# AnastasiaBelenkii/tendermint

Hardware: AMD Instinct MI355X
Metric: ed25519 verifies/sec at 1/2/4/8 GPUs + p50 VerifyCommit latency, 150 vals (higher is better)
Workload: dtype int32

## Files before the change

__graft_entry__.py:

```python
import os
import subprocess
import sys

REPO = os.path.dirname(os.path.abspath(__file__))


def build() -> None:
    env = dict(os.environ, PYTORCH_ROCM_ARCH="gfx950")
    subprocess.run(["make", "-s", "-C", os.path.join(REPO, "tendermint_amd", "csrc")], check=True, env=env)
    subprocess.run(["bash", os.path.join(REPO, "tools", "build_checks.sh")], check=True, env=env)
    subprocess.run(["make", "-s", "-C", os.path.join(REPO, "oracle")], check=True)
    subprocess.run(["make", "-s", "-C", os.path.join(REPO, "tendermint_amd", "testing", "csrc")], check=True)
    subprocess.run(["make", "-s", "-C", os.path.join(REPO, "tests", "native")], check=True)
    subprocess.run(["make", "-s", "-C", os.path.join(REPO, "tests", "native", "secp")], check=True)
    subprocess.run(["make", "-s", "-C", os.path.join(REPO, "tests", "native", "secpcomb")], check=True)
    subprocess.run(["make", "-s", "-C", os.path.join(REPO, "tests", "native", "merkle")], check=True)
    subprocess.run(["make", "-s", "-C", os.path.join(REPO, "tests", "native", "pcache")], check=True)
    subprocess.run(["make", "-s", "-C", os.path.join(REPO, "tests", "native", "colorder")], check=True)
    subprocess.run(["make", "-s", "-C", os.path.join(REPO, "tests", "native", "split")], check=True)
    subprocess.run(["make", "-s", "-C", os.path.join(REPO, "tests", "native", "blocks")], check=True)
    subprocess.run(["make", "-s", "-C", os.path.join(REPO, "tests", "native", "voteext")], check=True)
    subprocess.run(["make", "-s", "-C", os.path.join(REPO, "tests", "native", "proofops")], check=True)
    subprocess.run(["make", "-s", "-C", os.path.join(REPO, "tests", "native", "stage")], check=True)
    subprocess.run(["make", "-s", "-C", os.path.join(REPO, "tests", "native", "results")], check=True)
    subprocess.run(["make", "-s", "-C", os.path.join(REPO, "tests", "native", "keyorder")], check=True)
    subprocess.run(["make", "-s", "-C", os.path.join(REPO, "tests", "native", "blockwire")], check=True)
    subprocess.run(["make", "-s", "-C", os.path.join(REPO, "tests", "native", "lightwire")], check=True)
    subprocess.run(["make", "-s", "-C", os.path.join(REPO, "tests", "native", "valset")], check=True)
    sys.path.insert(0, REPO)
    import tendermint_amd
    from tendermint_amd import _native
    _native.lib()


def smoke() -> None:
    sys.path.insert(0, REPO)
    sys.path.insert(0, os.path.join(REPO, "oracle"))
    import numpy as np
    import torch
    from tendermint_amd import _native
    from tendermint_amd.testing.factory import make_c2_batch
    import oracle_c

    assert torch.cuda.is_available(), "smoke() needs a GPU"
    ctx = _native.Context(1)
    b = make_c2_batch(1000, seed=7)
    ok_g, vec_g = ctx.ed25519_verify_batch(b.pk, b.sig, b.msg, b.off)
    ok_o, vec_o = oracle_c.ed25519_verify_packed(b.pk, b.sig, b.msg, b.off, threads=4)
    assert ok_g == ok_o and np.array_equal(vec_g, vec_o), "GPU validity vector differs from the oracle"
    info = _native.build_info()
    print(f"smoke ok: {int(vec_g.sum())}/{b.n} valid, bit-exact vs oracle; {info['version']} "
          f"(src digest of this tree {'matches' if info['src_match'] else 'DIFFERS: ' + info['src_digest_tree']})")


if __name__ == "__main__":
    build()
    smoke()
```

tendermint_amd/csrc/verify_kernels.hip:

```cpp
#include <hip/hip_runtime.h>
#include <cstdlib>
#include <cstring>
#include <atomic>
#include "ed25519_core.h"
#include "quad.h"
#include "sr25519_core.h"
#include "verify_kernels.h"
#include "kernel_util.h"
#include "comb.h"
#include "halfscalar.h"
#include "ktimer.h"

namespace tmv {

__global__ void __launch_bounds__(kVerifyBlock)
k_ed25519_verify(const uint8_t *__restrict__ pk, const uint8_t *__restrict__ sig,
                 const uint8_t *__restrict__ msg, const uint32_t *__restrict__ msg_off, uint32_t n,
                 const ge_precomp *__restrict__ btable, uint8_t *__restrict__ valid, int aligned) {
  const uint32_t i = blockIdx.x * blockDim.x + threadIdx.x;
  if (i >= n) return;
  uint32_t a_w[8], r_w[8], s_w[8];
  if (aligned) {
    load_words_aligned(a_w, pk + 32ull * i);
    load_words_aligned(r_w, sig + 64ull * i);
    load_words_aligned(s_w, sig + 64ull * i + 32);
  } else {
    load_words_unaligned(a_w, pk + 32ull * i);
    load_words_unaligned(r_w, sig + 64ull * i);
    load_words_unaligned(s_w, sig + 64ull * i + 32);
  }
  const uint32_t o0 = msg_off[i], o1 = msg_off[i + 1];
  const bool ok = ed25519_verify_core(a_w, r_w, s_w, msg + o0, o1 - o0, btable);
  valid[i] = ok ? 1 : 0;
}


template <bool SR>
__device__ __forceinline__ void prep_store_point(uint32_t e, bool isA, bool ok, ge_p3 &P, const Ed25519Work &w) {
  if (!ok) ge_p3_identity(P);
  w.flags[4 * e + (isA ? 0 : 1)] = ok ? 1 : 0;
  if (w.niels) {
    niels_pt np;
    fe t;
    fe_sub(t, P.Y, P.X); fe_carry(np.ypx, t);
    fe_add(t, P.Y, P.X); fe_carry(np.ymx, t);
    fe_mul(t, P.T, consts::d2()); fe_neg(np.xy2d, t);
    np.pad[0] = np.pad[1] = 0;
    niels_store(w.niels, 2ull * e + (isA ? 1 : 0), np);
  }
  fe *dst = (isA ? w.negA : w.Rc) + 4ull * e;
  if (isA || SR) {
    fe t;
    if (isA) fe_neg(t, P.X); else t = P.X;
    dst[0] = t;
    dst[1] = P.Y;
    fe_one(t); dst[2] = t;
    if (isA) fe_neg(t, P.T); else t = P.T;
    dst[3] = t;
  } else {
    ge_cached c;
    ge_p3_to_cached(c, P);
    fe t;
    fe_carry(t, c.YmX); dst[0] = t;
    fe_carry(t, c.YpX); dst[1] = t;
    dst[2] = c.T2d;
    dst[3] = c.Z;
  }
}

template <bool SR>
__device__ __forceinline__ void prep_decode_block(uint32_t bx, const uint8_t *__restrict__ pk,
                                                  const uint8_t *__restrict__ sig, const uint32_t *__restrict__ idx,
                                                  const uint32_t *count_ptr, uint32_t n, Ed25519Work w, int aligned) {
  const uint32_t m = entry_count(count_ptr, n);
  const uint32_t j = bx * blockDim.x + threadIdx.x;
  if (j >= 2 * m) return;
  const bool isA = j < m;
  const uint32_t e = isA ? j : j - m;
  const uint32_t i = idx ? idx[e] : e;
  uint32_t p_w[8];
  const uint8_t *src = isA ? pk + 32ull * i : sig + 64ull * i;
  if (aligned) load_words_aligned(p_w, src);
  else load_words_unaligned(p_w, src);
  ge_p3 P;
  bool ok;
  if (SR) ok = ristretto_decode(P, p_w);
  else ok = ge_decode_zip215(P, p_w);
  prep_store_point<SR>(e, isA, ok, P, w);
}

template <bool SR>
__device__ __forceinline__ void prep_hash_block(uint32_t bx, const uint8_t *__restrict__ pk,
                                                const uint8_t *__restrict__ sig, const uint8_t *__restrict__ msg,
                                                const uint32_t *__restrict__ msg_off, const uint32_t *__restrict__ idx,
                                                const uint32_t *count_ptr, uint32_t n, Ed25519Work w,
                                                const strobe_t *__restrict__ prefix, int aligned) {
  const uint32_t m = entry_count(count_ptr, n);
  const uint32_t e = bx * blockDim.x + threadIdx.x;
  if (e >= m) return;
  const uint32_t i = idx ? idx[e] : e;
  uint32_t a_w[8], r_w[8];
  if (aligned) {
    load_words_aligned(a_w, pk + 32ull * i);
    load_words_aligned(r_w, sig + 64ull * i);
  } else {
    load_words_unaligned(a_w, pk + 32ull * i);
    load_words_unaligned(r_w, sig + 64ull * i);
  }
  uint32_t k[8];
  const uint32_t o0 = msg_off[i], o1 = msg_off[i + 1];
  if constexpr (SR) {
    __shared__ uint64_t strobe_lanes[25][kVerifyBlock];
    sr25519_challenge_lds<kVerifyBlock>(k, *prefix, &strobe_lanes[0][threadIdx.x], a_w, r_w, msg + o0, o1 - o0);
  } else {
    uint32_t h[16];
    sha512_pq_msg(h, r_w, a_w, msg + o0, o1 - o0);
    sc_reduce512(k, h);
  }
  uint4 *kd = reinterpret_cast<uint4 *>(w.k + 8ull * e);
  kd[0] = make_uint4(k[0], k[1], k[2], k[3]);
  kd[1] = make_uint4(k[4], k[5], k[6], k[7]);
  if (w.hs) {
    uint32_t u[4], v[4];
    bool neg = false;
    const bool fast = half::reduce(u, neg, v, k);
    uint4 *hd = reinterpret_cast<uint4 *>(w.hs + 12ull * e);
    hd[0] = make_uint4(u[0], u[1], u[2], u[3]);
    hd[1] = make_uint4(v[0], v[1], v[2], v[3]);
    hd[2] = make_uint4((fast ? 1u : 0u) | (neg ? 2u : 0u), 0u, 0u, 0u);
  }
}

template <bool SR>
__global__ void __launch_bounds__(kVerifyBlock)
k_prep_fused(const uint8_t *__restrict__ pk, const uint8_t *__restrict__ sig, const uint8_t *__restrict__ msg,
             const uint32_t *__restrict__ msg_off, const uint32_t *__restrict__ idx, const uint32_t *count_ptr,
             uint32_t n, Ed25519Work w, const strobe_t *__restrict__ prefix, int aligned, uint32_t dblocks) {
  if (blockIdx.x < dblocks) prep_decode_block<SR>(blockIdx.x, pk, sig, idx, count_ptr, n, w, aligned);
  else prep_hash_block<SR>(blockIdx.x - dblocks, pk, sig, msg, msg_off, idx, count_ptr, n, w, prefix, aligned);
}

__global__ void __launch_bounds__(kVerifyBlock)
k_prep_probe(const uint8_t *__restrict__ pk, const uint8_t *__restrict__ sig, const uint8_t *__restrict__ msg,
             const uint32_t *__restrict__ msg_off, const uint32_t *__restrict__ idx, uint32_t n, Ed25519Work w,
             int aligned, uint32_t rblocks, uint32_t hblocks) {
  if (blockIdx.x < rblocks) {
    const uint32_t e = blockIdx.x * blockDim.x + threadIdx.x;
    if (e >= n) return;
    const uint32_t i = idx ? idx[e] : e;
    uint32_t r_w[8];
    if (aligned) load_words_aligned(r_w, sig + 64ull * i);
    else load_words_unaligned(r_w, sig + 64ull * i);
    ge_p3 P;
    const bool ok = ge_decode_zip215(P, r_w);
    prep_store_point<false>(e, false, ok, P, w);
    return;
  }
  if (blockIdx.x < rblocks + hblocks) {
    prep_hash_block<false>(blockIdx.x - rblocks, pk, sig, msg, msg_off, idx, nullptr, n, w, nullptr, aligned);
    return;
  }
  const uint32_t e = (blockIdx.x - rblocks - hblocks) * blockDim.x + threadIdx.x;
  const bool live = e < n;
  bool hit = false;
  if (live) {
    const uint32_t i = idx ? idx[e] : e;
    uint32_t a_w[8];
    if (aligned) load_words_aligned(a_w, pk + 32ull * i);
    else load_words_unaligned(a_w, pk + 32ull * i);
    ge_p3 P;
    hit = pc_probe(P, w.pc.table, w.pc.bucket_mask, a_w);
    if (hit) prep_store_point<false>(e, true, true, P, w);
  }
  const uint32_t lane = threadIdx.x & 63;
  const uint64_t hm = __ballot(hit), mm = __ballot(live && !hit);
  uint32_t base = 0;
  if (lane == 0) {
    if (hm) atomicAdd(&w.pc.counters[0], (unsigned long long)__popcll(hm));
    if (mm) {
      atomicAdd(&w.pc.counters[1], (unsigned long long)__popcll(mm));
      base = atomicAdd(w.miss_count, (uint32_t)__popcll(mm));
    }
  }
  if (mm) {
    base = __shfl(base, 0);
    if (live && !hit) w.miss_list[base + __popcll(mm & ((1ull << lane) - 1))] = e;
  }
}

constexpr int kMissBlock = 64;
__global__ void __launch_bounds__(kMissBlock)
k_prep_miss(const uint8_t *__restrict__ pk, const uint32_t *__restrict__ idx, uint32_t n, Ed25519Work w,
            int aligned) {
  const uint32_t cnt = min(*w.miss_count, n);
  if (blockIdx.x * kMissBlock >= cnt) return;
  const uint32_t t = blockIdx.x * kMissBlock + threadIdx.x;
  if (t >= cnt) return;
  const uint32_t e = w.miss_list[t];
  if (e >= n) return;
  const uint32_t i = idx ? idx[e] : e;
  uint32_t a_w[8];
  if (aligned) load_words_aligned(a_w, pk + 32ull * i);
  else load_words_unaligned(a_w, pk + 32ull * i);
  ge_p3 P;
  const bool ok = ge_decode_zip215(P, a_w);
  if (ok) pc_insert(w.pc.table, w.pc.bucket_mask, a_w, P.X);
  prep_store_point<false>(e, true, ok, P, w);
}

constexpr int kQuadSigs = kQuadBlock / 4;

constexpr int kDigV = 0, kDigB = 64, kDigU = 96, kDigBytes = 128;

TMV_DEV void quad_multiples(fe *tab, const fe &P) {
  const int c = threadIdx.x & 3;
  fe r, Pm, Q, Q0;
  quad::to_cached(Q0, P);
  tab[0 * 4 + c] = Q0;
  quad::dbl(r, P);
  quad::p1p1_to_p3(Pm, r);
  quad::to_cached(Q, Pm);
  tab[1 * 4 + c] = Q;
  for (int t = 2; t < 8; t++) {
    quad::add(r, Pm, Q0);
    quad::p1p1_to_p3(Pm, r);
    quad::to_cached(Q, Pm);
    tab[t * 4 + c] = Q;
  }
}

template <bool SR>
TMV_DEV void neg_r_p3(fe &P, const fe &Rc) {
  const int c = threadIdx.x & 3;
  if (SR) {
    if (c == 0 || c == 3) fe_neg(P, Rc);
    else P = Rc;
    return;
  }
  fe o, t, K;
  quad::fe_dpp<quad::qp(1, 0, 3, 2)>(o, Rc);
  if (c == 0) fe_sub(t, Rc, o);
  else if (c == 1) fe_add(t, Rc, o);
  else t = o;
  if (c == 3) {
    const uint32_t w[8] = {0x323607aau, 0xda1f0d89u, 0xbd86abd1u, 0xf4a22967u,
                           0x32463099u, 0xd4e9deebu, 0xeb2a31bcu, 0x3f6f812du};
    fe_from_words(K, w);
  } else {
    fe_zero(K);
    K.v[0] = c == 2 ? 2 : 1;
  }
  quad::qmul(P, t, K);
}

template <bool SR, bool GT>
__device__ __forceinline__ void quad_block(uint32_t blk, fe *tab_lds, int8_t (*dig)[kDigBytes],
                                           const uint8_t *__restrict__ sig, const uint32_t *__restrict__ idx,
                                           const uint32_t *count_ptr, uint32_t n, const Ed25519Work &w,
                                           const fe *__restrict__ btab_q, uint8_t *__restrict__ out, int aligned,
                                           const uint8_t *__restrict__ group_ok, uint32_t group_log2,
                                           const uint8_t *__restrict__ sub_ok,
                                           const uint32_t *__restrict__ fail_list,
                                           const uint32_t *__restrict__ fail_count,
                                           const uint32_t *__restrict__ fb_list, uint32_t nl, int half_on) {
  const uint32_t m = entry_count(count_ptr, n);
  const int c = threadIdx.x & 3;
  const int q = threadIdx.x >> 2;
  uint32_t b0 = 0, e;
  bool live;
  if (fb_list) {
    if (blk * kQuadSigs >= nl) return;
    const uint32_t t = blk * kQuadSigs + q;
    live = t < nl;
    e = fb_list[live ? t : nl - 1];
  } else {
    if (fail_list) {
      const uint32_t per_log2 = group_log2 - 4;
      if (blk >= (*fail_count << per_log2)) return;
      b0 = (fail_list[blk >> per_log2] << group_log2) + ((blk & ((1u << per_log2) - 1)) << 4);
    } else {
      b0 = blk * kQuadSigs;
    }
    if (b0 >= m) return;
    const uint32_t raw = b0 + q;
    live = raw < m;
    e = live ? raw : m - 1;
  }
  const uint32_t i = idx ? idx[e] : e;
  bool pass = false;
  if (group_ok && !fb_list) {
    pass = !fail_list && group_ok[b0 >> group_log2];
    if (!pass && sub_ok) {
      pass = true;
      for (uint32_t s = b0 >> kSubGroupLog2; s <= (b0 + kQuadSigs - 1) >> kSubGroupLog2; s++) pass = pass && sub_ok[s];
    }
  }
  if (pass) {
    if (!live || c != 0) return;
    uint32_t s_raw[8], s_w[8];
    if (aligned) load_words_aligned(s_raw, sig + 64ull * i + 32);
    else load_words_unaligned(s_raw, sig + 64ull * i + 32);
    bool s_ok;
    if (SR) {
      s_ok = sr25519_decode_s(s_w, s_raw);
    } else {
      s_ok = sc_is_canonical(s_raw);
    }
    const bool a_ok = w.flags[4 * e] != 0;
    const bool r_ok = w.flags[4 * e + 1] != 0;
    const int status = SR ? (!a_ok ? -1 : (!s_ok ? -2 : (r_ok ? 1 : 0))) : ((a_ok && r_ok && s_ok) ? 1 : 0);
    out[i] = (uint8_t)(int8_t)status;
    return;
  }

  uint32_t s_raw[8], s_w[8];
  if (aligned) load_words_aligned(s_raw, sig + 64ull * i + 32);
  else load_words_unaligned(s_raw, sig + 64ull * i + 32);
  bool s_ok;
  if (SR) {
    s_ok = sr25519_decode_s(s_w, s_raw);
  } else {
#pragma unroll
    for (int t = 0; t < 8; t++) s_w[t] = s_raw[t];
    s_ok = sc_is_canonical(s_w);
  }
  if (!s_ok) s_w[7] &= 0x0fffffffu;
  bool fast, neg_u;
  {
    uint32_t k_w[8];
    const uint4 *kp = reinterpret_cast<const uint4 *>(w.k + 8ull * e);
    const uint4 k0 = kp[0], k1 = kp[1];
    k_w[0] = k0.x; k_w[1] = k0.y; k_w[2] = k0.z; k_w[3] = k0.w;
    k_w[4] = k1.x; k_w[5] = k1.y; k_w[6] = k1.z; k_w[7] = k1.w;
    half::Scalars sc;
    if (half_on == 1 && w.hs) {
      const uint4 *hp = reinterpret_cast<const uint4 *>(w.hs + 12ull * e);
      const uint4 hu = hp[0], hv = hp[1], hf = hp[2];
      const uint32_t u4[4] = {hu.x, hu.y, hu.z, hu.w}, v4[4] = {hv.x, hv.y, hv.z, hv.w};
      half::scalars_from(sc, u4, (hf.x & 2u) != 0, v4, (hf.x & 1u) != 0, k_w, s_w);
    } else if (half_on == 1 || (half_on == 2 && e % 3 != 0)) {
      half::scalars(sc, k_w, s_w);
    } else {
#pragma unroll
      for (int t = 0; t < 8; t++) { sc.u[t] = t == 0; sc.v[t] = k_w[t]; sc.b[t] = s_w[t]; }
      sc.fast = false;
      sc.u_neg = false;
    }
    fast = sc.fast;
    neg_u = sc.u_neg;
    if (c == 0) {
      if (fast) recode16_n<32>(&dig[q][kDigV], sc.v);
      else recode16_n<64>(&dig[q][kDigV], sc.v);
    } else if (c == 1) {
      recode256_store(&dig[q][kDigB], sc.b);
    } else if (c == 2) {
      recode16_n<32>(&dig[q][kDigU], sc.u);
    }
  }
  const bool a_ok = w.flags[4 * e] != 0;
  const bool r_ok = w.flags[4 * e + 1] != 0;

  fe *tabA = GT ? w.tabA + 64ull * e : tab_lds + q * 64;
  fe *tabR = tabA + 32;
  quad_multiples(tabA, w.negA[4ull * e + c]);
  {
    fe nR;
    neg_r_p3<SR>(nR, w.Rc[4ull * e + c]);
    quad_multiples(tabR, nR);
  }
  __syncthreads();

  fe acc, r;
  quad::p3_identity(acc);
  fe idq;
  quad::cached_identity(idq);
  const int nw = fast ? 32 : 64;
  const int nw_wave = __ballot(!fast) ? 64 : 32;
  const fe *btab_hi = btab_q + 4 * kBaseQuadEntries;
  for (int wdx = nw_wave - 1; wdx >= 0; wdx--) {
    if (wdx >= nw) continue;
    const bool even = (wdx & 1) == 0;
    const int da = dig[q][kDigV + wdx];
    const int du = wdx < 32 ? dig[q][kDigU + wdx] : 0;
    const int db = even ? dig[q][kDigB + (wdx >> 1)] : 0;
    const int dh = (even && fast) ? dig[q][kDigB + 16 + (wdx >> 1)] : 0;
    const int aa = da < 0 ? -da : da, au = du < 0 ? -du : du, ab = db < 0 ? -db : db, ah = dh < 0 ? -dh : dh;
    fe aent = tabA[(aa ? aa - 1 : 0) * 4 + c];
    fe rent = tabR[(au ? au - 1 : 0) * 4 + c];
    fe bent, hent;
    if (even) {
      bent = btab_q[(ab ? ab - 1 : 0) * 4 + c];
      if (fast) hent = btab_hi[(ah ? ah - 1 : 0) * 4 + c];
    }
    if (wdx != nw - 1) {
#pragma unroll
      for (int d = 0; d < 4; d++) {
        quad::dbl(r, acc);
        quad::p1p1_to_p3(acc, r);
      }
    }
    fe_cmov(aent, idq, aa == 0);
    quad::cached_cneg(aent, da < 0);
    quad::add(r, acc, aent);
    quad::p1p1_to_p3(acc, r);
    if (wdx < 32) {
      fe_cmov(rent, idq, au == 0);
      quad::cached_cneg(rent, (du < 0) != neg_u);
      quad::add(r, acc, rent);
      quad::p1p1_to_p3(acc, r);
    }
    if (even) {
      fe_cmov(bent, idq, ab == 0);
      quad::cached_cneg(bent, (db < 0) != neg_u);
      quad::add(r, acc, bent);
      quad::p1p1_to_p3(acc, r);
      if (fast) {
        fe_cmov(hent, idq, ah == 0);
        quad::cached_cneg(hent, (dh < 0) != neg_u);
        quad::add(r, acc, hent);
        quad::p1p1_to_p3(acc, r);
      }
    }
  }
  int status;
  if (SR) {
    const bool eq = quad::is_ristretto_identity(acc);
    status = !a_ok ? -1 : (!s_ok ? -2 : (!r_ok ? 0 : (eq ? 1 : 0)));
  } else {
    const bool ok = quad::is_identity_times8(acc) && s_ok && a_ok && r_ok;
    status = ok ? 1 : 0;
  }
  if (live && c == 0) out[i] = (uint8_t)(int8_t)status;
}


template <bool SR, bool GT>
__global__ void __launch_bounds__(kQuadBlock)
k_verify_quad(const uint8_t *__restrict__ sig, const uint32_t *__restrict__ idx, const uint32_t *count_ptr,
              uint32_t n, Ed25519Work w, const fe *__restrict__ btab_q, uint8_t *__restrict__ out, int aligned,
              const uint8_t *__restrict__ group_ok, uint32_t group_log2, const uint8_t *__restrict__ sub_ok,
              const uint32_t *__restrict__ fail_list, const uint32_t *__restrict__ fail_count,
              const uint32_t *__restrict__ fb_list, const uint32_t *__restrict__ fb_count, int half_on) {
  __shared__ fe tab_lds[GT ? 4 : kQuadSigs * 16 * 4];
  __shared__ int8_t dig[kQuadSigs][kDigBytes];
  quad_block<SR, GT>(blockIdx.x, tab_lds, dig, sig, idx, count_ptr, n, w, btab_q, out, aligned, group_ok,
                     group_log2, sub_ok, fail_list, fail_count, fb_list, fb_list ? *fb_count : 0u, half_on);
}

template <bool SR>
__global__ void __launch_bounds__(kQuadBlock)
k_verify_quad_list(const uint8_t *__restrict__ sig, const uint32_t *__restrict__ idx, const uint32_t *count_ptr,
                   uint32_t n, Ed25519Work w, const fe *__restrict__ btab_q, uint8_t *__restrict__ out,
                   int aligned, const uint32_t *__restrict__ fb_list, const uint32_t *__restrict__ fb_count,
                   int half_on) {
  __shared__ fe tab_lds[4];
  __shared__ int8_t dig[kQuadSigs][kDigBytes];
  const uint32_t nl = *fb_count;
  for (uint32_t blk = blockIdx.x; blk * kQuadSigs < nl; blk += gridDim.x) {
    quad_block<SR, true>(blk, tab_lds, dig, sig, idx, count_ptr, n, w, btab_q, out, aligned, nullptr, 0u, nullptr,
                         nullptr, nullptr, fb_list, nl, half_on);
    __syncthreads();
  }
}

__global__ void __launch_bounds__(256)
k_partition(const uint8_t *__restrict__ kind, uint32_t n, uint32_t *counts, uint32_t *idx_ed,
            uint32_t *idx_sr, uint8_t *__restrict__ out) {
  __shared__ uint32_t wcnt[2][4];
  __shared__ uint32_t base[2];
  const uint32_t i = blockIdx.x * 256 + threadIdx.x;
  const uint32_t lane = threadIdx.x & 63, wave = threadIdx.x >> 6;
  const bool in = i < n;
  const uint8_t k = in ? kind[i] : 255;
  if (in && k > 1) out[i] = 0;
  const uint64_t b0 = __ballot(k == 0), b1 = __ballot(k == 1);
  const uint64_t below = lane ? (~0ull >> (64 - lane)) : 0ull;
  if (lane == 0) {
    wcnt[0][wave] = (uint32_t)__popcll(b0);
    wcnt[1][wave] = (uint32_t)__popcll(b1);
  }
  __syncthreads();
  if (threadIdx.x < 2) {
    const uint32_t t = threadIdx.x;
    base[t] = atomicAdd(&counts[t], wcnt[t][0] + wcnt[t][1] + wcnt[t][2] + wcnt[t][3]);
  }
  __syncthreads();
  if (k > 1) return;
  uint32_t at = base[k] + (uint32_t)__popcll((k == 0 ? b0 : b1) & below);
  for (uint32_t w = 0; w < wave; w++) at += wcnt[k][w];
  (k == 0 ? idx_ed : idx_sr)[at] = i;
}

__global__ void __launch_bounds__(256)
k_partition_range(const uint8_t *__restrict__ kind, uint32_t lo, uint32_t hi, uint32_t base_ed, uint32_t base_sr,
                  uint32_t *cursor, uint32_t *counts, uint32_t *idx_ed, uint32_t *idx_sr, uint8_t *out) {
  __shared__ uint32_t wcnt[2][4];
  __shared__ uint32_t base[2];
  const uint32_t i = lo + blockIdx.x * 256 + threadIdx.x;
  const uint32_t lane = threadIdx.x & 63, wave = threadIdx.x >> 6;
  const bool in = i < hi;
  const uint8_t k = in ? kind[i] : 255;
  if (in && k > 1) out[i] = 0;
  const uint64_t b0 = __ballot(k == 0), b1 = __ballot(k == 1);
  const uint64_t below = lane ? (~0ull >> (64 - lane)) : 0ull;
  if (lane == 0) {
    wcnt[0][wave] = (uint32_t)__popcll(b0);
    wcnt[1][wave] = (uint32_t)__popcll(b1);
  }
  __syncthreads();
  if (threadIdx.x < 2) {
// ... 219 lines not shown
  __shared__ fe part[2][kQuadSigs][4];
  __shared__ fe Rs[kQuadSigs][4];
  __shared__ uint8_t rok[kQuadSigs];
  const uint32_t base = blockIdx.x * kQuadSigs;
  if (base >= n) return;
  const int wave = threadIdx.x >> 6;
  const int lane = threadIdx.x & 63;
  if (wave == 1) {
    if (lane < kQuadSigs) {
      const uint32_t i = min(base + lane, n - 1);
      uint32_t r_w[8];
      if (aligned) load_words_aligned(r_w, sig + 64ull * i);
      else load_words_unaligned(r_w, sig + 64ull * i);
      ge_p3 P;
      const bool ok = SR ? ristretto_decode(P, r_w) : ge_decode_zip215(P, r_w);
      if (!ok) ge_p3_identity(P);
      rok[lane] = ok ? 1 : 0;
      if (SR) {
        Rs[lane][0] = P.X; Rs[lane][1] = P.Y;
        fe t; fe_one(t); Rs[lane][2] = t;
        Rs[lane][3] = P.T;
      } else {
        ge_cached cc;
        ge_p3_to_cached(cc, P);
        fe t;
        fe_carry(t, cc.YmX); Rs[lane][0] = t;
        fe_carry(t, cc.YpX); Rs[lane][1] = t;
        Rs[lane][2] = cc.T2d;
        Rs[lane][3] = cc.Z;
      }
    }
    __syncthreads();
    return;
  }
  const int c = lane & 3;
  const int q = lane >> 2;
  const uint32_t raw = base + q;
  const bool live = raw < n;
  const uint32_t i = live ? raw : n - 1;
  fe acc, r, idq;
  quad::p3_identity(acc);
  quad::cached_identity(idq);
  if (wave == 2) {
    uint32_t s_raw[8], s_w[8];
    if (aligned) load_words_aligned(s_raw, sig + 64ull * i + 32);
    else load_words_unaligned(s_raw, sig + 64ull * i + 32);
    bool s_ok;
    if (SR) {
      s_ok = sr25519_decode_s(s_w, s_raw);
    } else {
#pragma unroll
      for (int t = 0; t < 8; t++) s_w[t] = s_raw[t];
      s_ok = sc_is_canonical(s_w);
    }
    if (!s_ok) s_w[7] &= 0x0fffffffu;
    if (c == 1) recode256_store(&dig_s[q][0], s_w);
    __builtin_amdgcn_fence(__ATOMIC_RELEASE, "workgroup");
    __builtin_amdgcn_wave_barrier();
    __builtin_amdgcn_fence(__ATOMIC_ACQUIRE, "workgroup");
    auto entry_at = [&](int t, int &dsg) -> const fe * {
      dsg = dig_s[q][t];
      const int a = dsg < 0 ? -dsg : dsg;
      return bcomb + ((t * kBaseQuadEntries) + (a ? a - 1 : 0)) * 4 + c;
    };
    comb_accumulate<32>(acc, idq, entry_at);
    part[0][q][c] = acc;
    __syncthreads();
    return;
  }
  const int h = wave == 3 ? 1 : 0;
  if (c == 0) {
    uint32_t k_w[8];
    uint32_t a_w[8], r_w[8];
    if (aligned) {
      load_words_aligned(a_w, pk + 32ull * i);
      load_words_aligned(r_w, sig + 64ull * i);
    } else {
      load_words_unaligned(a_w, pk + 32ull * i);
      load_words_unaligned(r_w, sig + 64ull * i);
    }
    const uint32_t o0 = msg_off[i], o1 = msg_off[i + 1];
    if constexpr (SR) {
      __shared__ uint64_t strobe_lanes[2][25][kQuadSigs];
      sr25519_challenge_lds<kQuadSigs>(k_w, *prefix, &strobe_lanes[h][0][q], a_w, r_w, msg + o0, o1 - o0);
    } else {
      uint32_t hh[16];
      sha512_pq_msg(hh, r_w, a_w, msg + o0, o1 - o0);
      sc_reduce512(k_w, hh);
    }
    recode16_store(&dig_k[h][q][0], k_w, true);
  }
  __builtin_amdgcn_fence(__ATOMIC_RELEASE, "workgroup");
  __builtin_amdgcn_wave_barrier();
  __builtin_amdgcn_fence(__ATOMIC_ACQUIRE, "workgroup");
  const uint32_t slot = key_slot[i];
  const fe *krow = kt.tab + (size_t)slot * kKeyRowsEntries * 4;
  auto entry_at = [&](int t, int &dsg) -> const fe * {
    const int tt = t + 32 * h;
    dsg = dig_k[h][q][tt];
    const int a = dsg < 0 ? -dsg : dsg;
    return krow + ((tt * 8) + (a ? a - 1 : 0)) * 4 + c;
  };
  comb_accumulate<32>(acc, idq, entry_at);
  if (wave == 3) {
    part[1][q][c] = acc;
    __syncthreads();
    return;
  }
  uint32_t s_raw[8], s_w[8];
  if (aligned) load_words_aligned(s_raw, sig + 64ull * i + 32);
  else load_words_unaligned(s_raw, sig + 64ull * i + 32);
  bool s_ok;
  if (SR) {
    s_ok = sr25519_decode_s(s_w, s_raw);
  } else {
#pragma unroll
    for (int t = 0; t < 8; t++) s_w[t] = s_raw[t];
    s_ok = sc_is_canonical(s_w);
  }
  const bool a_ok = kt.ok[slot] != 0;
  __syncthreads();
#pragma unroll
  for (int pi = 0; pi < 2; pi++) {
    fe pc;
    quad::to_cached(pc, part[pi][q][c]);
    quad::add(r, acc, pc);
    quad::p1p1_to_p3(acc, r);
  }
  const bool r_ok = rok[q] != 0;
  int status;
  if (SR) {
    const fe Rq = Rs[q][c];
    const bool eq = quad::ristretto_equal(acc, Rq);
    status = !a_ok ? -1 : (!s_ok ? -2 : (!r_ok ? 0 : (eq ? 1 : 0)));
  } else {
    fe Rq = Rs[q][c];
    quad::cached_cneg(Rq, true);
    quad::add(r, acc, Rq);
    quad::p1p1_to_p3(acc, r);
    status = (quad::is_identity_times8(acc) && s_ok && a_ok && r_ok) ? 1 : 0;
  }
  if (live && c == 0) out[i] = (uint8_t)(int8_t)status;
}

hipError_t launch_key_build(bool sr, const uint8_t *keys, const uint32_t *slots, uint32_t m, KeyTable kt,
                            fe *bases, hipStream_t stream) {
  if (m == 0) return hipSuccess;
  const uint32_t blocks = (m + kQuadSigs - 1) / kQuadSigs;
  if (sr) hipLaunchKernelGGL(k_key_bases<true>, dim3(blocks), dim3(kQuadBlock), 0, stream, keys, slots, m, kt, bases);
  else hipLaunchKernelGGL(k_key_bases<false>, dim3(blocks), dim3(kQuadBlock), 0, stream, keys, slots, m, kt, bases);
  hipError_t e = hipGetLastError();
  if (e != hipSuccess) return e;
  const uint32_t rblocks = (uint32_t)((64ull * m + kQuadSigs - 1) / kQuadSigs);
  hipLaunchKernelGGL(k_key_rows, dim3(rblocks), dim3(kQuadBlock), 0, stream, slots, m, kt, (const fe *)bases);
  return hipGetLastError();
}

hipError_t launch_verify_cached(bool sr, const uint8_t *pk, const uint8_t *sig, const uint8_t *msg,
                                const uint32_t *msg_off, const uint32_t *key_slot, uint32_t n, KeyTable kt,
                                const fe *bcomb, const strobe_t *prefix, Ed25519Work w, uint8_t *out,
                                uint32_t fused_max, hipStream_t stream) {
  if (n == 0) return hipSuccess;
  const int aligned = ((((uintptr_t)pk) | ((uintptr_t)sig)) & 15) == 0;
  if (n <= fused_max) {
    const uint32_t blocks = (n + kQuadSigs - 1) / kQuadSigs;
    if (sr) hipLaunchKernelGGL(k_verify_cached_fused4<true>, dim3(blocks), dim3(4 * kQuadBlock), 0, stream, pk, sig,
                               msg, msg_off, key_slot, n, kt, bcomb, prefix, out, aligned);
    else hipLaunchKernelGGL(k_verify_cached_fused4<false>, dim3(blocks), dim3(4 * kQuadBlock), 0, stream, pk, sig,
                            msg, msg_off, key_slot, n, kt, bcomb, prefix, out, aligned);
    return hipGetLastError();
  }
  w.niels = nullptr;
  const uint32_t pblocks = (uint32_t)((2ull * n + kVerifyBlock - 1) / kVerifyBlock);
  if (sr) hipLaunchKernelGGL(k_prep_cached<true>, dim3(pblocks), dim3(kVerifyBlock), 0, stream, pk, sig, msg, msg_off, nullptr, n, w, prefix, aligned);
  else hipLaunchKernelGGL(k_prep_cached<false>, dim3(pblocks), dim3(kVerifyBlock), 0, stream, pk, sig, msg, msg_off, nullptr, n, w, prefix, aligned);
  hipError_t e = hipGetLastError();
  if (e != hipSuccess) return e;
  const uint32_t qblocks = (n + kQuadSigs - 1) / kQuadSigs;
  if (sr) hipLaunchKernelGGL(k_verify_comb<true>, dim3(qblocks), dim3(kQuadBlock), 0, stream, sig, key_slot, nullptr, n, w, kt, bcomb, out,
                             aligned, nullptr, 0u);
  else hipLaunchKernelGGL(k_verify_comb<false>, dim3(qblocks), dim3(kQuadBlock), 0, stream, sig, key_slot, nullptr, n, w, kt, bcomb, out,
                          aligned, nullptr, 0u);
  return hipGetLastError();
}

template <bool SR>
hipError_t launch_prep_cached(const uint8_t *pk, const uint8_t *sig, const uint8_t *msg, const uint32_t *msg_off,
                              const uint32_t *idx, uint32_t n, const strobe_t *prefix, Ed25519Work w, int aligned,
                              hipStream_t stream) {
  const uint32_t pblocks = (uint32_t)((2ull * n + kVerifyBlock - 1) / kVerifyBlock);
  hipLaunchKernelGGL(k_prep_cached<SR>, dim3(pblocks), dim3(kVerifyBlock), 0, stream, pk, sig, msg, msg_off, idx, n, w,
                     prefix, aligned);
  return hipGetLastError();
}
template hipError_t launch_prep_cached<false>(const uint8_t *, const uint8_t *, const uint8_t *, const uint32_t *,
                                              const uint32_t *, uint32_t, const strobe_t *, Ed25519Work, int,
                                              hipStream_t);
template hipError_t launch_prep_cached<true>(const uint8_t *, const uint8_t *, const uint8_t *, const uint32_t *,
                                             const uint32_t *, uint32_t, const strobe_t *, Ed25519Work, int,
                                             hipStream_t);

template <bool SR>
hipError_t launch_comb_fallback(const uint8_t *sig, const uint32_t *key_slot, const uint32_t *idx, uint32_t n,
                                Ed25519Work w, KeyTable kt, const fe *bcomb, uint8_t *out, int aligned,
                                const uint8_t *group_ok, uint32_t group_log2, hipStream_t stream) {
  const uint32_t qblocks = (n + kQuadSigs - 1) / kQuadSigs;
  hipLaunchKernelGGL(k_verify_comb<SR>, dim3(qblocks), dim3(kQuadBlock), 0, stream, sig, key_slot, idx, n, w, kt, bcomb,
                     out, aligned, group_ok, group_log2);
  return hipGetLastError();
}
template hipError_t launch_comb_fallback<false>(const uint8_t *, const uint32_t *, const uint32_t *, uint32_t,
                                                Ed25519Work, KeyTable, const fe *, uint8_t *, int, const uint8_t *,
                                                uint32_t, hipStream_t);
template hipError_t launch_comb_fallback<true>(const uint8_t *, const uint32_t *, const uint32_t *, uint32_t,
                                               Ed25519Work, KeyTable, const fe *, uint8_t *, int, const uint8_t *,
                                               uint32_t, hipStream_t);

static std::atomic<int> g_half_mode{1};
void set_half_scalar_mode(int mode) { g_half_mode = mode == 0 || mode == 2 ? mode : 1; }
static int half_scalars_on() { return g_half_mode.load(std::memory_order_relaxed); }

template <bool SR>
static void launch_quad(uint32_t qblocks, hipStream_t stream, const uint8_t *sig, const uint32_t *idx,
                        const uint32_t *count_ptr, uint32_t n, Ed25519Work w, const fe *btab_q, uint8_t *out,
                        int aligned, const uint8_t *group_ok, uint32_t group_log2,
                        const uint8_t *sub_ok = nullptr, const uint32_t *fail_list = nullptr,
                        const uint32_t *fail_count = nullptr, const uint32_t *fb_list = nullptr,
                        const uint32_t *fb_count = nullptr, bool fallback = false) {
  const int half = half_scalars_on();
  const bool global = fallback || qblocks > 3u * 256u;
  if (global)
    hipLaunchKernelGGL((k_verify_quad<SR, true>), dim3(qblocks), dim3(kQuadBlock), 0, stream, sig, idx, count_ptr, n,
                       w, btab_q, out, aligned, group_ok, group_log2, sub_ok, fail_list, fail_count, fb_list,
                       fb_count, half);
  else
    hipLaunchKernelGGL((k_verify_quad<SR, false>), dim3(qblocks), dim3(kQuadBlock), 0, stream, sig, idx, count_ptr, n,
                       w, btab_q, out, aligned, group_ok, group_log2, sub_ok, fail_list, fail_count, fb_list,
                       fb_count, half);
}

static int is_aligned(const void *a, const void *b) {
  return ((((uintptr_t)a) | ((uintptr_t)b)) & 15) == 0;
}

template <bool SR>
static hipError_t launch_pipeline(const uint8_t *pk, const uint8_t *sig, const uint8_t *msg,
                                  const uint32_t *msg_off, const uint32_t *idx, const uint32_t *count_ptr,
                                  uint32_t n, const fe *btab_q, const strobe_t *prefix, Ed25519Work w,
                                  uint8_t *out, hipStream_t stream) {
  if (n == 0) return hipSuccess;
  const int aligned = is_aligned(pk, sig);
  w.hs = w.hs_buf;
  hipError_t e = launch_prep<SR>(pk, sig, msg, msg_off, idx, count_ptr, n, prefix, w, aligned, stream);
  if (e != hipSuccess) return e;
  const uint32_t qblocks = (n + kQuadSigs - 1) / kQuadSigs;
  launch_quad<SR>(qblocks, stream, sig, idx, count_ptr, n, w, btab_q, out, aligned, nullptr, 0u);
  return hipGetLastError();
}

template <bool SR>
hipError_t launch_quad_fallback(const uint8_t *sig, const uint32_t *idx, const uint32_t *count_ptr, uint32_t n,
                                const fe *btab_q, Ed25519Work w, const uint8_t *group_ok, uint32_t group_log2,
                                uint8_t *out, int aligned, hipStream_t stream, const uint8_t *sub_ok,
                                const uint32_t *fail_list, const uint32_t *fail_count, const uint32_t *fb_list,
                                const uint32_t *fb_count) {
  const uint32_t qblocks = fb_list ? (n + kQuadSigs - 1) / kQuadSigs
                           : fail_list ? ((((n + (1u << group_log2) - 1) >> group_log2)) << (group_log2 - 4))
                                       : (n + kQuadSigs - 1) / kQuadSigs;
  if (fb_list) {
    const uint32_t grid = qblocks < 256u * 16u ? qblocks : 256u * 16u;
    hipLaunchKernelGGL(k_verify_quad_list<SR>, dim3(grid), dim3(kQuadBlock), 0, stream, sig, idx, count_ptr, n, w,
                       btab_q, out, aligned, fb_list, fb_count, half_scalars_on());
    return hipGetLastError();
  }
  launch_quad<SR>(qblocks, stream, sig, idx, count_ptr, n, w, btab_q, out, aligned, group_ok, group_log2, sub_ok,
                  fail_list, fail_count, fb_list, fb_count, true);
  return hipGetLastError();
}
template hipError_t launch_quad_fallback<false>(const uint8_t *, const uint32_t *, const uint32_t *, uint32_t,
                                                const fe *, Ed25519Work, const uint8_t *, uint32_t, uint8_t *, int,
                                                hipStream_t, const uint8_t *, const uint32_t *, const uint32_t *,
                                                const uint32_t *, const uint32_t *);
template hipError_t launch_quad_fallback<true>(const uint8_t *, const uint32_t *, const uint32_t *, uint32_t,
                                               const fe *, Ed25519Work, const uint8_t *, uint32_t, uint8_t *, int,
                                               hipStream_t, const uint8_t *, const uint32_t *, const uint32_t *,
                                               const uint32_t *, const uint32_t *);

static std::atomic<uint32_t> g_point_cache_min{kPointCacheMin};
void set_point_cache_min(uint32_t n) { g_point_cache_min = n ? n : kPointCacheMin; }
uint32_t point_cache_min() { return g_point_cache_min.load(std::memory_order_relaxed); }

template <bool SR>
hipError_t launch_prep(const uint8_t *pk, const uint8_t *sig, const uint8_t *msg, const uint32_t *msg_off,
                       const uint32_t *idx, const uint32_t *count_ptr, uint32_t n, const strobe_t *prefix,
                       Ed25519Work w, int aligned, hipStream_t stream) {
  const uint32_t dblocks = (uint32_t)((2ull * n + kVerifyBlock - 1) / kVerifyBlock);
  const uint32_t hblocks = (n + kVerifyBlock - 1) / kVerifyBlock;
  const bool cached = !SR && w.niels && !count_ptr && w.pc.table && w.miss_list && n >= w.pc.min_n;
  void *tk = ktimer::begin(ktimer::kPrep, stream);
  hipError_t e;
  if (cached) {
    e = hipMemsetAsync(w.miss_count, 0, sizeof(uint32_t), stream);
    if (e == hipSuccess) {
      hipLaunchKernelGGL(k_prep_probe, dim3(3 * hblocks), dim3(kVerifyBlock), 0, stream, pk, sig, msg, msg_off, idx,
                         n, w, aligned, hblocks, hblocks);
      e = hipGetLastError();
    }
    if (e == hipSuccess) {
      hipLaunchKernelGGL(k_prep_miss, dim3((n + kMissBlock - 1) / kMissBlock), dim3(kMissBlock), 0, stream, pk, idx, n,
                         w, aligned);
      e = hipGetLastError();
    }
  } else {
    hipLaunchKernelGGL(k_prep_fused<SR>, dim3(dblocks + hblocks), dim3(kVerifyBlock), 0, stream, pk, sig, msg, msg_off,
                       idx, count_ptr, n, w, prefix, aligned, dblocks);
    e = hipGetLastError();
  }
  ktimer::end(tk, stream);
  return e;
}
template hipError_t launch_prep<false>(const uint8_t *, const uint8_t *, const uint8_t *, const uint32_t *,
                                       const uint32_t *, const uint32_t *, uint32_t, const strobe_t *, Ed25519Work,
                                       int, hipStream_t);
template hipError_t launch_prep<true>(const uint8_t *, const uint8_t *, const uint8_t *, const uint32_t *,
                                      const uint32_t *, const uint32_t *, uint32_t, const strobe_t *, Ed25519Work,
                                      int, hipStream_t);

hipError_t launch_ed25519_verify_quad(const uint8_t *pk, const uint8_t *sig, const uint8_t *msg,
                                      const uint32_t *msg_off, uint32_t n, const fe *btab_q, Ed25519Work w,
                                      uint8_t *valid, hipStream_t stream) {
  return launch_pipeline<false>(pk, sig, msg, msg_off, nullptr, nullptr, n, btab_q, nullptr, w, valid, stream);
}

hipError_t launch_sr25519_verify_quad(const uint8_t *pk, const uint8_t *sig, const uint8_t *msg,
                                      const uint32_t *msg_off, uint32_t n, const fe *btab_q, const strobe_t *prefix,
                                      Ed25519Work w, int8_t *status, hipStream_t stream) {
  return launch_pipeline<true>(pk, sig, msg, msg_off, nullptr, nullptr, n, btab_q, prefix, w,
                               reinterpret_cast<uint8_t *>(status), stream);
}

hipError_t launch_mixed_verify(const uint8_t *kind, const uint8_t *pk, const uint8_t *sig, const uint8_t *msg,
                               const uint32_t *msg_off, uint32_t n, const fe *btab_q, const strobe_t *prefix,
                               Ed25519Work w_ed, Ed25519Work w_sr, uint32_t *counts, uint32_t *idx_ed,
                               uint32_t *idx_sr, int8_t *status, hipStream_t stream) {
  if (n == 0) return hipSuccess;
  hipError_t e = hipMemsetAsync(counts, 0, 2 * sizeof(uint32_t), stream);
  if (e != hipSuccess) return e;
  uint8_t *out = reinterpret_cast<uint8_t *>(status);
  hipLaunchKernelGGL(k_partition, dim3((n + 255) / 256), dim3(256), 0, stream, kind, n, counts, idx_ed, idx_sr, out);
  if ((e = hipGetLastError()) != hipSuccess) return e;
  e = launch_pipeline<false>(pk, sig, msg, msg_off, idx_ed, counts, n, btab_q, prefix, w_ed, out, stream);
  if (e != hipSuccess) return e;
  return launch_pipeline<true>(pk, sig, msg, msg_off, idx_sr, counts + 1, n, btab_q, prefix, w_sr, out, stream);
}

hipError_t launch_partition_range(const uint8_t *kind, uint32_t lo, uint32_t hi, uint32_t base_ed, uint32_t base_sr,
                                  uint32_t *cursor, uint32_t *counts, uint32_t *idx_ed, uint32_t *idx_sr, uint8_t *out,
                                  hipStream_t stream) {
  if (hi <= lo) return hipSuccess;
  hipLaunchKernelGGL(k_partition_range, dim3((hi - lo + 255) / 256), dim3(256), 0, stream, kind, lo, hi, base_ed,
                     base_sr, cursor, counts, idx_ed, idx_sr, out);
  return hipGetLastError();
}

hipError_t launch_partition(const uint8_t *kind, uint32_t n, uint32_t *counts, uint32_t *idx_ed, uint32_t *idx_sr,
                            uint8_t *out, hipStream_t stream) {
  hipError_t e = hipMemsetAsync(counts, 0, 2 * sizeof(uint32_t), stream);
  if (e != hipSuccess) return e;
  hipLaunchKernelGGL(k_partition, dim3((n + 255) / 256), dim3(256), 0, stream, kind, n, counts, idx_ed, idx_sr, out);
  return hipGetLastError();
}

hipError_t launch_ed25519_verify(const uint8_t *pk, const uint8_t *sig, const uint8_t *msg,
                                 const uint32_t *msg_off, uint32_t n, const ge_precomp *btable,
                                 uint8_t *valid, hipStream_t stream) {
  if (n == 0) return hipSuccess;
  const int aligned = ((((uintptr_t)pk) | ((uintptr_t)sig)) & 15) == 0;
  const uint32_t blocks = (n + kVerifyBlock - 1) / kVerifyBlock;
  hipLaunchKernelGGL(k_ed25519_verify, dim3(blocks), dim3(kVerifyBlock), 0, stream, pk, sig, msg, msg_off, n,
                     btable, valid, aligned);
  return hipGetLastError();
}

}
```

Measured before the change: 248.1 million.

## Probe point cache in per-thread chunks, merging runs of identical public keys

```diff
diff --git a/__graft_entry__.py b/__graft_entry__.py
--- a/__graft_entry__.py
+++ b/__graft_entry__.py
@@ -16,6 +16,7 @@
     subprocess.run(["make", "-s", "-C", os.path.join(REPO, "tests", "native", "secpcomb")], check=True)
     subprocess.run(["make", "-s", "-C", os.path.join(REPO, "tests", "native", "merkle")], check=True)
     subprocess.run(["make", "-s", "-C", os.path.join(REPO, "tests", "native", "pcache")], check=True)
+    subprocess.run(["make", "-s", "-C", os.path.join(REPO, "tests", "native", "pchunk")], check=True)
     subprocess.run(["make", "-s", "-C", os.path.join(REPO, "tests", "native", "colorder")], check=True)
     subprocess.run(["make", "-s", "-C", os.path.join(REPO, "tests", "native", "split")], check=True)
     subprocess.run(["make", "-s", "-C", os.path.join(REPO, "tests", "native", "blocks")], check=True)
diff --git a/tendermint_amd/csrc/probe_chunk.h b/tendermint_amd/csrc/probe_chunk.h
--- /dev/null
+++ b/tendermint_amd/csrc/probe_chunk.h
@@ -0,0 +1,57 @@
+#pragma once
+#include <cstdint>
+#include "curve25519.h"
+
+namespace tmv {
+
+#ifndef TMV_PROBE_CHUNK
+#define TMV_PROBE_CHUNK 16
+#endif
+constexpr uint32_t kProbeChunk = TMV_PROBE_CHUNK;
+static_assert(kProbeChunk >= 1 && kProbeChunk <= 32 && (kProbeChunk & (kProbeChunk - 1)) == 0,
+              "kProbeChunk: a power of two <= 32 (a part view starts at a multiple of 32; k fits 5 bits)");
+
+constexpr uint32_t kProbeSlotBits = 27;
+constexpr uint32_t kProbeMaxPacked = 1u << kProbeSlotBits;
+
+TMV_HD bool probe_chunk_merges(uint32_t n) { return n <= kProbeMaxPacked; }
+
+TMV_HD bool probe_key_equal(const uint32_t a[8], const uint32_t b[8]) {
+  uint32_t diff = 0;
+#pragma unroll
+  for (int i = 0; i < 8; i++) diff |= a[i] ^ b[i];
+  return diff == 0;
+}
+
+template <class Load>
+TMV_HD uint32_t probe_chunk_plan(uint32_t cnt, bool merge, Load load) {
+  if (cnt == 0) return 0;
+  uint32_t reps = 1, prev[8], cur[8];
+  load(0u, prev);
+  for (uint32_t t = 1; t < cnt; t++) {
+    load(t, cur);
+    if (!merge || !probe_key_equal(cur, prev)) reps |= 1u << t;
+#pragma unroll
+    for (int i = 0; i < 8; i++) prev[i] = cur[i];
+  }
+  return reps;
+}
+
+TMV_HD uint32_t probe_ctz(uint32_t x) {
+#if defined(__HIP_DEVICE_COMPILE__)
+  return (uint32_t)__ffs((int)x) - 1;
+#else
+  return (uint32_t)__builtin_ctz(x);
+#endif
+}
+TMV_HD uint32_t probe_chunk_followers(uint32_t reps, uint32_t cnt, uint32_t t) {
+  const uint32_t above = t + 1 < 32 ? reps >> (t + 1) : 0;
+  const uint32_t next = above ? t + 1 + probe_ctz(above) : cnt;
+  return next - t - 1;
+}
+
+TMV_HD uint32_t probe_miss_pack(uint32_t e, uint32_t k) { return e | (k << kProbeSlotBits); }
+TMV_HD uint32_t probe_miss_slot(uint32_t word, bool merge) { return merge ? word & (kProbeMaxPacked - 1) : word; }
+TMV_HD uint32_t probe_miss_followers(uint32_t word, bool merge) { return merge ? word >> kProbeSlotBits : 0; }
+
+}
diff --git a/tendermint_amd/csrc/verify_kernels.hip b/tendermint_amd/csrc/verify_kernels.hip
--- a/tendermint_amd/csrc/verify_kernels.hip
+++ b/tendermint_amd/csrc/verify_kernels.hip
@@ -10,6 +10,7 @@
 #include "comb.h"
 #include "halfscalar.h"
 #include "ktimer.h"
+#include "probe_chunk.h"
 
 namespace tmv {
 
@@ -35,37 +36,49 @@
 }
 
 
-template <bool SR>
-__device__ __forceinline__ void prep_store_point(uint32_t e, bool isA, bool ok, ge_p3 &P, const Ed25519Work &w) {
+struct prep_words {
+  niels_pt np;
+  fe q[4];
+};
+template <bool SR>
+__device__ __forceinline__ void prep_point_words(prep_words &o, bool isA, bool ok, ge_p3 &P, bool niels) {
   if (!ok) ge_p3_identity(P);
-  w.flags[4 * e + (isA ? 0 : 1)] = ok ? 1 : 0;
-  if (w.niels) {
-    niels_pt np;
+  if (niels) {
     fe t;
-    fe_sub(t, P.Y, P.X); fe_carry(np.ypx, t);
-    fe_add(t, P.Y, P.X); fe_carry(np.ymx, t);
-    fe_mul(t, P.T, consts::d2()); fe_neg(np.xy2d, t);
-    np.pad[0] = np.pad[1] = 0;
-    niels_store(w.niels, 2ull * e + (isA ? 1 : 0), np);
-  }
-  fe *dst = (isA ? w.negA : w.Rc) + 4ull * e;
+    fe_sub(t, P.Y, P.X); fe_carry(o.np.ypx, t);
+    fe_add(t, P.Y, P.X); fe_carry(o.np.ymx, t);
+    fe_mul(t, P.T, consts::d2()); fe_neg(o.np.xy2d, t);
+    o.np.pad[0] = o.np.pad[1] = 0;
+  }
   if (isA || SR) {
-    fe t;
-    if (isA) fe_neg(t, P.X); else t = P.X;
-    dst[0] = t;
-    dst[1] = P.Y;
-    fe_one(t); dst[2] = t;
-    if (isA) fe_neg(t, P.T); else t = P.T;
-    dst[3] = t;
+    if (isA) fe_neg(o.q[0], P.X); else o.q[0] = P.X;
+    o.q[1] = P.Y;
+    fe_one(o.q[2]);
+    if (isA) fe_neg(o.q[3], P.T); else o.q[3] = P.T;
   } else {
     ge_cached c;
     ge_p3_to_cached(c, P);
-    fe t;
-    fe_carry(t, c.YmX); dst[0] = t;
-    fe_carry(t, c.YpX); dst[1] = t;
-    dst[2] = c.T2d;
-    dst[3] = c.Z;
-  }
+    fe_carry(o.q[0], c.YmX);
+    fe_carry(o.q[1], c.YpX);
+    o.q[2] = c.T2d;
+    o.q[3] = c.Z;
+  }
+}
+__device__ __forceinline__ void prep_write_words(uint32_t e, bool isA, bool ok, const prep_words &o,
+                                                 const Ed25519Work &w) {
+  w.flags[4 * e + (isA ? 0 : 1)] = ok ? 1 : 0;
+  if (w.niels) niels_store(w.niels, 2ull * e + (isA ? 1 : 0), o.np);
+  fe *dst = (isA ? w.negA : w.Rc) + 4ull * e;
+  dst[0] = o.q[0];
+  dst[1] = o.q[1];
+  dst[2] = o.q[2];
+  dst[3] = o.q[3];
+}
+template <bool SR>
+__device__ __forceinline__ void prep_store_point(uint32_t e, bool isA, bool ok, ge_p3 &P, const Ed25519Work &w) {
+  prep_words o;
+  prep_point_words<SR>(o, isA, ok, P, w.niels != nullptr);
+  prep_write_words(e, isA, ok, o, w);
 }
 
 template <bool SR>
@@ -140,6 +153,22 @@
   else prep_hash_block<SR>(blockIdx.x - dblocks, pk, sig, msg, msg_off, idx, count_ptr, n, w, prefix, aligned);
 }
 
+__device__ __forceinline__ void prep_load_key(uint32_t a_w[8], const uint8_t *__restrict__ pk,
+                                              const uint32_t *__restrict__ idx, uint32_t e, int aligned) {
+  const uint32_t i = idx ? idx[e] : e;
+  if (aligned) load_words_aligned(a_w, pk + 32ull * i);
+  else load_words_unaligned(a_w, pk + 32ull * i);
+}
+
+__device__ __forceinline__ uint32_t wave_scan_incl(uint32_t v, uint32_t lane) {
+#pragma unroll
+  for (uint32_t d = 1; d < 64; d <<= 1) {
+    const uint32_t t = __shfl_up(v, d);
+    if (lane >= d) v += t;
+  }
+  return v;
+}
+
 __global__ void __launch_bounds__(kVerifyBlock)
 k_prep_probe(const uint8_t *__restrict__ pk, const uint8_t *__restrict__ sig, const uint8_t *__restrict__ msg,
              const uint32_t *__restrict__ msg_off, const uint32_t *__restrict__ idx, uint32_t n, Ed25519Work w,
@@ -160,31 +189,44 @@
     prep_hash_block<false>(blockIdx.x - rblocks, pk, sig, msg, msg_off, idx, nullptr, n, w, nullptr, aligned);
     return;
   }
-  const uint32_t e = (blockIdx.x - rblocks - hblocks) * blockDim.x + threadIdx.x;
-  const bool live = e < n;
-  bool hit = false;
-  if (live) {
-    const uint32_t i = idx ? idx[e] : e;
+  const uint64_t c0 = ((uint64_t)(blockIdx.x - rblocks - hblocks) * blockDim.x + threadIdx.x) * kProbeChunk;
+  const uint32_t e0 = c0 < n ? (uint32_t)c0 : n;
+  const uint32_t cnt = min(kProbeChunk, n - e0);
+  const bool merge = probe_chunk_merges(n);
+  const uint32_t reps =
+      probe_chunk_plan(cnt, merge, [&](uint32_t t, uint32_t key[8]) { prep_load_key(key, pk, idx, e0 + t, aligned); });
+  uint32_t hits = 0, missed = 0;
+  for (uint32_t todo = reps; todo != 0; todo &= todo - 1) {
+    const uint32_t t = probe_ctz(todo), k = probe_chunk_followers(reps, cnt, t);
     uint32_t a_w[8];
-    if (aligned) load_words_aligned(a_w, pk + 32ull * i);
-    else load_words_unaligned(a_w, pk + 32ull * i);
+    prep_load_key(a_w, pk, idx, e0 + t, aligned);
     ge_p3 P;
-    hit = pc_probe(P, w.pc.table, w.pc.bucket_mask, a_w);
-    if (hit) prep_store_point<false>(e, true, true, P, w);
+    if (pc_probe(P, w.pc.table, w.pc.bucket_mask, a_w)) {
+      prep_words o;
+      prep_point_words<false>(o, true, true, P, w.niels != nullptr);
+      for (uint32_t j = 0; j <= k; j++) prep_write_words(e0 + t + j, true, true, o, w);
+      hits += 1 + k;
+    } else {
+      missed |= 1u << t;
+    }
   }
   const uint32_t lane = threadIdx.x & 63;
-  const uint64_t hm = __ballot(hit), mm = __ballot(live && !hit);
+  const uint32_t nm = __popc(missed);
+  const uint32_t words_incl = wave_scan_incl(nm, lane);
+  const uint32_t ent = __shfl(wave_scan_incl(hits | ((cnt - hits) << 16), lane), 63);
+  const uint32_t words = __shfl(words_incl, 63);
   uint32_t base = 0;
   if (lane == 0) {
-    if (hm) atomicAdd(&w.pc.counters[0], (unsigned long long)__popcll(hm));
-    if (mm) {
-      atomicAdd(&w.pc.counters[1], (unsigned long long)__popcll(mm));
-      base = atomicAdd(w.miss_count, (uint32_t)__popcll(mm));
-    }
-  }
-  if (mm) {
-    base = __shfl(base, 0);
-    if (live && !hit) w.miss_list[base + __popcll(mm & ((1ull << lane) - 1))] = e;
+    if (ent & 0xffffu) atomicAdd(&w.pc.counters[0], (unsigned long long)(ent & 0xffffu));
+    if (ent >> 16) atomicAdd(&w.pc.counters[1], (unsigned long long)(ent >> 16));
+    if (words) base = atomicAdd(w.miss_count, words);
+  }
+  if (words) {
+    uint32_t at = __shfl(base, 0) + words_incl - nm;
+    for (uint32_t m = missed; m != 0; m &= m - 1) {
+      const uint32_t t = probe_ctz(m);
+      w.miss_list[at++] = merge ? probe_miss_pack(e0 + t, probe_chunk_followers(reps, cnt, t)) : e0 + t;
+    }
   }
 }
 
@@ -196,16 +238,19 @@
   if (blockIdx.x * kMissBlock >= cnt) return;
   const uint32_t t = blockIdx.x * kMissBlock + threadIdx.x;
   if (t >= cnt) return;
-  const uint32_t e = w.miss_list[t];
+  const bool merge = probe_chunk_merges(n);
+  const uint32_t word = w.miss_list[t];
+  const uint32_t e = probe_miss_slot(word, merge);
   if (e >= n) return;
-  const uint32_t i = idx ? idx[e] : e;
+  const uint32_t k = min(probe_miss_followers(word, merge), n - 1 - e);
   uint32_t a_w[8];
-  if (aligned) load_words_aligned(a_w, pk + 32ull * i);
-  else load_words_unaligned(a_w, pk + 32ull * i);
+  prep_load_key(a_w, pk, idx, e, aligned);
   ge_p3 P;
   const bool ok = ge_decode_zip215(P, a_w);
   if (ok) pc_insert(w.pc.table, w.pc.bucket_mask, a_w, P.X);
-  prep_store_point<false>(e, true, ok, P, w);
+  prep_words o;
+  prep_point_words<false>(o, true, ok, P, w.niels != nullptr);
+  for (uint32_t j = 0; j <= k; j++) prep_write_words(e + j, true, ok, o, w);
 }
 
 constexpr int kQuadSigs = kQuadBlock / 4;
@@ -1031,8 +1076,9 @@
   if (cached) {
     e = hipMemsetAsync(w.miss_count, 0, sizeof(uint32_t), stream);
     if (e == hipSuccess) {
-      hipLaunchKernelGGL(k_prep_probe, dim3(3 * hblocks), dim3(kVerifyBlock), 0, stream, pk, sig, msg, msg_off, idx,
-                         n, w, aligned, hblocks, hblocks);
+      const uint32_t pblocks = ((n + kProbeChunk - 1) / kProbeChunk + kVerifyBlock - 1) / kVerifyBlock;
+      hipLaunchKernelGGL(k_prep_probe, dim3(2 * hblocks + pblocks), dim3(kVerifyBlock), 0, stream, pk, sig, msg,
+                         msg_off, idx, n, w, aligned, hblocks, hblocks);
       e = hipGetLastError();
     }
     if (e == hipSuccess) {
```

Result: slower. 243.9 million (-1.7%).
